# Parcels-code/Parcels

Hardware: AMD Instinct MI355X
Metric: RK4 particle-steps/sec (higher is better)
Workload: dtype f64

## Files before the change

### parcels_amd/csrc/pk_api.hip

```cpp
#include <hip/hip_runtime.h>

#include <algorithm>
#include <array>
#include <chrono>
#include <cmath>
#include <cstdio>
#include <cstdlib>
#include <cstring>
#include <string>
#include <thread>
#include <vector>

#include <rocprim/rocprim.hpp>

#include "pk_hashbuild.h"
#include "pk_neighbors.h"
#include "pk_interact.h"
#include "pk_density.h"
#include "pk_connectivity.h"
#include "pk_host_stage.h"
#include "pk_kernels.h"
#include "pk_ux.h"
#include "pk_sigma.h"

// ... 101 lines not shown
    DCounters* d_counters = nullptr;
    char *d_desc = nullptr, *h_desc = nullptr;
    size_t desc_bytes = 0;
    unsigned long long* d_summary = nullptr;
    void* stage[PK_STAGE_BUFFERS] = {};
    size_t stage_bytes[PK_STAGE_BUFFERS] = {};
    size_t stage_chunk = 0;
    hipEvent_t stage_ev[PK_STAGE_BUFFERS] = {};
    int stage_next = 0;
    double stage_fill_s = 0, stage_wait_s = 0, stage_bytes_total = 0;
    hipDeviceProp_t prop;
    bool in_flight = false;
    int fl_launches = 0;
    int fl_program = 0;
    bool rerun_valid = false;
    pk_exec_params rerun_prm{};
    void (*user_launch)(const void*, int32_t, int32_t, int32_t, uint64_t, void*) = nullptr;
    int32_t user_flags = 0;
    int32_t user_nsample = 0;
    int32_t user_sample_fid[4] = {0, 0, 0, 0};
    char* d_chk = nullptr;
    size_t chk_bytes = 0;
    bool chk_valid = false, chk_has_perm = false;
    int64_t chk_n = 0;
    bool fl_sorted = false;
    int64_t fl_n = 0;
    DCounters* h_counters = nullptr;
    DCounters h_counters0;
    unsigned long long* d_twe = nullptr;
    unsigned long long* d_twe_found = nullptr;
    unsigned int* d_twe_hit = nullptr;
    std::vector<int64_t> twe_found_host;
    std::vector<uint8_t> twe_hit_host;
    bool twe_overflow_host = false;
    int fl_twe_n = 0;
    std::vector<int64_t> rerun_keys;
    unsigned long long* h_summary = nullptr;
    unsigned long long* d_tstats = nullptr;
    unsigned long long* d_clk = nullptr;
    unsigned long long* h_clk = nullptr;
    double* d_sigma = nullptr;
    SigmaA sigma{};
    bool has_sigma = false;
    int sort_horizontal_major = -1;
    int no_special = 0;
    bool eval_points_f32 = false;
    int no_cell_cache = 0;
    int no_hash_dir = 0;
    int no_cell_table = 0;
    int no_fast = 0;
    int no_fast_cgrid = 0;
    bool no_block_cache = false;
    int block_cache = -1;
    int fast_grid = 0;
    struct Snapshot {
        void* dev[PK_NCOLS] = {};
        void* host[PK_NCOLS] = {};
        int64_t capacity = 0;
        int64_t n = 0;
        uint32_t mask = 0;
        int ngrids = 0;
        size_t ss = 0;
        size_t extra_elem[PK_MAX_EXTRA] = {};
        hipEvent_t ready = nullptr, done = nullptr;
        bool in_flight = false;
    } snap[2];
    CoordTable tab_a, tab_c;
    double* d_ct2 = nullptr;
    int ct2_grid = -1;
    int ct2_near = 0;
    char* d_vp = nullptr;
    size_t vp_bytes = 0;
    int vp_fU = -1, vp_fV = -1;
    std::vector<int32_t> vp_level;
    std::vector<uint64_t> vp_gen;
    int clock_probe = 0;
    bool fl_clock_probe = false;
    int no_velocity_pairs = 1;
    uint64_t upload_counter = 0;

    PkSelect sel;
    struct PkComm* comm = nullptr;
    pk::Neighbors* nbr = nullptr;
    pk::Interact* inter = nullptr;

    int32_t fail(const char* where, hipError_t e) {
        err = std::string(where) + ": " + hipGetErrorString(e);
        return -1;
    }
    int32_t fail(const std::string& msg) {
        err = msg;
        return -2;
    }
};

#define PK_HIP(ctx, call)                                  \
    do {                                                   \
        hipError_t e_ = (call);                            \
        if (e_ != hipSuccess) return (ctx)->fail(#call, e_); \
    } while (0)

namespace pk {

PK_DEV unsigned long long order_double(double v) {
    unsigned long long b = (unsigned long long)__double_as_longlong(v);
    return (b & 0x8000000000000000ull) ? ~b : (b | 0x8000000000000000ull);
// ... 402 lines not shown
    }
    pk_ctx* ctx = new pk_ctx();
    ctx->device = device;
    if (const char* e = getenv("PK_SORT_HORIZONTAL")) ctx->sort_horizontal_major = atoi(e);
    if (const char* e = getenv("PK_NO_SPECIAL")) ctx->no_special = atoi(e);
    if (const char* e = getenv("PK_NO_CELL_CACHE")) ctx->no_cell_cache = atoi(e);
    if (const char* e = getenv("PK_NO_HASH_DIR")) ctx->no_hash_dir = atoi(e);
    if (const char* e = getenv("PK_NO_CELL_TABLE")) ctx->no_cell_table = atoi(e);
    if (const char* e = getenv("PK_NO_FAST")) ctx->no_fast = atoi(e);
    if (const char* e = getenv("PK_NO_FAST_CGRID")) ctx->no_fast_cgrid = atoi(e);
    if (const char* e = getenv("PK_NO_VELOCITY_PAIRS")) ctx->no_velocity_pairs = atoi(e);
    if (const char* e = getenv("PK_VELOCITY_PAIRS")) ctx->no_velocity_pairs = !atoi(e);
    ctx->no_block_cache = getenv("PK_NO_BLOCK_CACHE") != nullptr;
    *out = ctx;
    PK_HIP(ctx, hipSetDevice(device));
    PK_HIP(ctx, hipGetDeviceProperties(&ctx->prop, device));
    PK_HIP(ctx, hipStreamCreateWithFlags(&ctx->compute, hipStreamNonBlocking));
    PK_HIP(ctx, hipStreamCreateWithFlags(&ctx->copy, hipStreamNonBlocking));
    PK_HIP(ctx, hipEventCreate(&ctx->ev0));
    PK_HIP(ctx, hipEventCreate(&ctx->ev1));
    PK_HIP(ctx, hipEventCreate(&ctx->ev2));
    PK_HIP(ctx, hipEventCreate(&ctx->ev_p0));
    PK_HIP(ctx, hipEventCreate(&ctx->ev_p1));
    for (int k = 0; k < PK_STAGE_BUFFERS; k++) PK_HIP(ctx, hipEventCreateWithFlags(&ctx->stage_ev[k], hipEventDisableTiming));
    PK_HIP(ctx, hipMalloc((void**)&ctx->d_counters, sizeof(DCounters)));
    PK_HIP(ctx, hipMalloc((void**)&ctx->d_twe, sizeof(unsigned long long) * PK_MAX_TWE));
    PK_HIP(ctx, hipMalloc((void**)&ctx->d_twe_found, sizeof(unsigned long long) * TWE_FOUND_SLOTS));
    PK_HIP(ctx, hipMalloc((void**)&ctx->d_twe_hit, sizeof(unsigned int) * PK_MAX_TWE));
    PK_HIP(ctx, hipMalloc((void**)&ctx->d_summary, sizeof(unsigned long long) * (PK_NUM_STATE_CODES + 2)));
    PK_HIP(ctx, hipHostMalloc((void**)&ctx->h_counters, sizeof(DCounters), hipHostMallocDefault));
    PK_HIP(ctx, hipHostMalloc((void**)&ctx->h_summary, sizeof(unsigned long long) * (PK_NUM_STATE_CODES + 2), hipHostMallocDefault));
    PK_HIP(ctx, hipMalloc((void**)&ctx->d_clk, sizeof(unsigned long long) * 32));
    PK_HIP(ctx, hipMalloc((void**)&ctx->d_tstats, sizeof(unsigned long long) * 3));
    PK_HIP(ctx, hipHostMalloc((void**)&ctx->h_clk, sizeof(unsigned long long) * 32, hipHostMallocDefault));
    return 0;
}

int32_t pk_set_option(pk_ctx* ctx, const char* name, int32_t value) {
    if (!ctx || !name) return -2;
    const std::string n(name);
    if (n == "fast_path") ctx->no_fast = !value;
    else if (n == "fast_cgrid") ctx->no_fast_cgrid = !value;
    else if (n == "velocity_pairs") ctx->no_velocity_pairs = !value;
    else if (n == "clock_probe") ctx->clock_probe = value;
    else if (n == "special_programs") ctx->no_special = !value;
    else if (n == "cell_cache") ctx->no_cell_cache = !value;
    else if (n == "hash_directory") ctx->no_hash_dir = !value;
    else if (n == "cell_table") ctx->no_cell_table = !value;
    else if (n == "sort_horizontal") ctx->sort_horizontal_major = value;
    else if (n == "eval_points_f32") ctx->eval_points_f32 = value != 0;
    else if (n == "block_cache") {
        if (value < -1 || value > 2) return ctx->fail("pk_set_option: block_cache is -1 (planned), 0 (none), 1 (stage-pair block) or 2 (level-pair cache)");
        ctx->block_cache = value;
    }
    else if (n == "fast_grid") {
        if (value < 0) return ctx->fail("pk_set_option: fast_grid is 0 (planned) or the largest number of workgroups of the persistent A-grid launch");
        ctx->fast_grid = value;
    }
    else return ctx->fail("pk_set_option: unknown option '" + n + "'");
    return 0;
}

int32_t pk_upload_stats(pk_ctx* ctx, double* out4) {
    if (!ctx || !out4) return -2;
    out4[0] = ctx->stage_fill_s;
    out4[1] = ctx->stage_wait_s;
    out4[2] = ctx->stage_bytes_total;
    out4[3] = (double)pkhost::copy_threads();
    return 0;
}

static void free_snapshots(pk_ctx* ctx) {
    for (auto& sn : ctx->snap) {
        if (sn.in_flight && sn.done) (void)hipEventSynchronize(sn.done);
        for (int k = 0; k < PK_NCOLS; k++) {
            if (sn.dev[k]) (void)hipFree(sn.dev[k]);
            if (sn.host[k]) (void)hipHostFree(sn.host[k]);
            sn.dev[k] = sn.host[k] = nullptr;
        }
        sn.capacity = 0;
        sn.in_flight = false;
    }
}

int32_t pk_destroy(pk_ctx* ctx) {
    if (!ctx) return 0;
    (void)hipSetDevice(ctx->device);
    (void)hipDeviceSynchronize();
    for (auto& g : ctx->grids)
        for (void* p : g.allocs) (void)hipFree(p);
    for (auto& f : ctx->fields) {
        if (f.dev_data && f.owns_data) (void)hipFree(f.dev_data);
        if (f.dev_time) (void)hipFree(f.dev_time);
    }
    free_particles(ctx);
    free_snapshots(ctx);
    for (auto& sn : ctx->snap) {
        if (sn.ready) (void)hipEventDestroy(sn.ready);
        if (sn.done) (void)hipEventDestroy(sn.done);
    }
    if (ctx->d_pack_tmp) (void)hipFree(ctx->d_pack_tmp);
    if (ctx->tab_a.d) (void)hipFree(ctx->tab_a.d);
    if (ctx->tab_c.d) (void)hipFree(ctx->tab_c.d);
    if (ctx->d_ct2) (void)hipFree(ctx->d_ct2);
    if (ctx->d_vp) (void)hipFree(ctx->d_vp);
    if (ctx->d_sigma) (void)hipFree(ctx->d_sigma);
// ... 1556 lines not shown
    const bool sigma_module = us.present && (us.flags & PK_USER_SIGMA);
    if (sigma_module && !croco && !ctx->has_sigma)
        return ctx->fail("the registered user program was built for the CROCO sigma loop: it runs a list on a context with CROCO parameters only (pk_set_croco)");
    if (croco || sigma_module) {
        if (!ctx->has_sigma) return ctx->fail("a CROCO kernel needs the CROCO parameters of the context (pk_set_croco)");
        if (us.present && !sigma_module)
            return ctx->fail("the registered user program was built for the kernel-list interpreter: a list with a CROCO kernel needs the sigma variant (PK_USER_SIGMA)");
        if (ctx_is_typed(ctx)) return ctx->fail("the CROCO kernels need float64 coordinate arrays");
        if (prm->interp_uv != 0 && prm->interp_uv != 1) return ctx->fail("the CROCO program interpolates the velocity with XLinear_Velocity or CGrid_Velocity");
        p.prog = PROG_SIGMA;
        p.lds = (size_t)ctx->sigma.n * 2 * sizeof(double);
        a.sigma = ctx->sigma;
        return 0;
    }
    bool rest_policy = true;
    for (int k = 1; k < prm->nk; k++)
        rest_policy = rest_policy && (prm->kernels[k] == PK_KERNEL_DELETE_ON_ERROR || prm->kernels[k] == PK_KERNEL_DELETE_OUT_OF_BOUNDS);
    if (rest_policy && use_lds) {
        if (prm->kernels[0] == PK_KERNEL_ADVECTION_RK4) p.prog = PROG_RK4;
        if (prm->kernels[0] == PK_KERNEL_ADVECTION_RK4_3D) p.prog = PROG_RK4_3D;
        if (prm->kernels[0] == PK_KERNEL_ADVECTION_RK45 && !ctx->no_special) p.prog = PROG_RK45;
        if (prm->kernels[0] == PK_KERNEL_ADVECTIONDIFFUSION_M1 && !ctx->no_special) p.prog = PROG_M1;
    }
    if (prm->body_only) p.prog = PROG_GENERIC;
    const bool typed = ctx_is_typed(ctx);
    if (typed) p.prog = PROG_TYPED;
    const bool curv = ctx->grids[a.main_grid].d.kind == 1;
    const bool listed = prm->twe_n > 0 && !us.assume_unlisted;
    const int ufast = (us.present && use_lds && !listed && !typed) ? user_fast_shape(prm, us.flags) : -1;
    const bool user_samples = us.nsample > 0 || (us.flags & (PK_USER_SAMPLES_UV | PK_USER_SAMPLES_UVW));
    int fast_prog = -1;
    const bool ride = ufast >= 0 && (!curv || !user_samples);
    if (ride) fast_prog = ufast ? PROG_RK4_3D : PROG_RK4;
    else if (!listed && (p.prog == PROG_RK4 || p.prog == PROG_RK4_3D || (curv && (p.prog == PROG_RK45 || p.prog == PROG_M1)))) fast_prog = p.prog;
    if (fast_prog < 0) return 0;
    if (!curv) {
        if (int32_t rc = fill_fast(ctx, prm, a, fast_prog)) return rc;
        if (ride && a.fast.ok && !fill_fast_scalars(ctx, prm, a.fast, us.nsample, us.fids)) a.fast.ok = 0;
        if (!a.fast.ok) return 0;
        p.kernel = fast_prog == PROG_RK4_3D ? DEDICATED_A3 : DEDICATED_A2;
        p.lds = (size_t)a.fast.lds_n * 2 * sizeof(double);
        const bool lp_kernel = fast_prog == PROG_RK4 && !ride;
        const size_t lp_lds = (p.lds + (size_t)FAST_LP_BYTES + 2047) / 2048 * 2048;
        const bool lp_fits = 2 * lp_lds <= (size_t)160 * 1024;
        int mode = ctx->block_cache;
        if (ctx->no_block_cache && mode != 2) mode = 0;
        if (mode == 2 && !(lp_kernel && lp_fits))
            return ctx->fail(!lp_kernel ? "block_cache 2: only the library's 2-D A-grid kernel (AdvectionRK4 without user kernels) has the level-pair cache"
                                        : "block_cache 2: the coordinate tables leave no room for the level-pair cache at 16 waves per CU");
        if (mode < 0) mode = lp_kernel && lp_fits ? 2 : 1;
        if (mode == 2) {
            p.lp = FAST_LP_CACHE;
            a.fast.lds_blk = a.fast.lds_n;
            p.lds += (size_t)FAST_LP_BYTES;
        } else if (mode == 0 && lp_kernel && !ctx->no_block_cache) {
            p.lp = FAST_LP_REGS;
            a.fast.lds_blk = 0;
        } else {
            const bool blk = mode == 1 && fast_prog != PROG_RK4_3D && p.lds + (size_t)FAST_BLK_BYTES <= 64 * 1024;
            a.fast.lds_blk = blk ? a.fast.lds_n : 0;
            if (blk) p.lds += (size_t)FAST_BLK_BYTES;
        }
    } else {
        if (int32_t rc = fill_fastc(ctx, prm, a, fast_prog, prm->have_guess0 || us.assume_guessed, p.lds)) return rc;
        if (!a.fastc.ok) return 0;
        p.kernel = fast_prog == PROG_RK4_3D ? DEDICATED_C3 : DEDICATED_C2;
    }
    p.prog = fast_prog;
    p.ride = ride;
    return 0;
}

static void launch_general(int prog, int field_f32, int curv, const pk_exec_params* prm, int use_lds, const KArgs& a, dim3 grid, size_t lds_bytes, hipStream_t s) {
    switch (prog) {
        case PROG_RK4: launch_program<PROG_RK4>(field_f32, curv, prm->interp_uv, use_lds, a, grid, lds_bytes, s); break;
        case PROG_RK4_3D: launch_program<PROG_RK4_3D>(field_f32, curv, prm->interp_uv, use_lds, a, grid, lds_bytes, s); break;
        case PROG_RK45: launch_program<PROG_RK45>(field_f32, curv, prm->interp_uv, use_lds, a, grid, lds_bytes, s); break;
        case PROG_M1: launch_program<PROG_M1>(field_f32, curv, prm->interp_uv, use_lds, a, grid, lds_bytes, s); break;
        case PROG_TYPED: launch_program<PROG_TYPED>(field_f32, curv, prm->interp_uv, use_lds, a, grid, lds_bytes, s); break;
        default: launch_program<PROG_GENERIC>(field_f32, curv, prm->interp_uv, use_lds, a, grid, lds_bytes, s); break;
    }
}

int32_t pk_execute_begin(pk_ctx* ctx, const pk_exec_params* prm) {
    if (!ctx || !prm) return -2;
    if (!ctx->bound) return ctx->fail("no particles bound");
    if (ctx->in_flight) return ctx->fail("pk_execute_begin: a launch is already in flight (call pk_execute_end)");
    if (prm->nk < 1 || prm->nk > PK_MAX_KERNELS) return ctx->fail("params.nk out of range");
    PK_HIP(ctx, hipSetDevice(ctx->device));
    ctx->fl_clock_probe = false;
    KArgs a;
    size_t lds_bytes = 0;
    int use_lds = 0;
    int32_t rc = launch_args(ctx, prm, a, lds_bytes, use_lds);
    if (rc) return rc;
    rc = upload_descriptors(ctx, a);
    if (rc) return rc;
    bool need_kh = false, has_user = false;
    for (int k = 0; k < prm->nk; k++) {
        const int id = prm->kernels[k];
        if (id == PK_KERNEL_ADVECTIONDIFFUSION_M1 || id == PK_KERNEL_ADVECTIONDIFFUSION_EM || id == PK_KERNEL_DIFFUSION_UNIFORM_KH)
            need_kh = true;
        if (id == PK_KERNEL_ADVECTION_RK45 && !ctx->dev.next_dt) return ctx->fail("AdvectionRK45 needs the next_dt column");
        if (id >= PK_KERNEL_USER0 && id < PK_KERNEL_USER0 + PK_MAX_USER_KERNELS) {
            has_user = true;
            if (!ctx->user_launch) return ctx->fail("a user kernel id without a registered program (pk_set_user_program)");
// ... 813 lines not shown
```

### parcels_amd/csrc/pk_device.h

```cpp
#pragma once
#include <hip/hip_runtime.h>
#include <stdint.h>

#include "../../include/parcels_hip.h"

namespace pk {

struct DGrid {
    int32_t kind, spherical;
    int32_t has_x, has_y, has_z;
    int32_t nx, ny, nz;
    int32_t xdim, ydim, zdim;
    int32_t off_x, off_y, off_z;
    int32_t lon_f32, lat_f32, depth_f32;
    int32_t h_bitwidth;
    double deg2m;
    const double* lon;
    const double* lat;
    const double* depth;
    const double* node_tab;
    const double* cell_tab;
    const uint32_t* h_keys;
    const int64_t* h_starts;
    const int64_t* h_counts;
// ... 21 lines not shown
};

struct DParticles {
    int64_t n;
    int32_t ngrids, spatial_f32;
    double* t;
    void *z, *y, *x, *dz, *dy, *dx;
    double* dt;
    double* next_dt;
    int32_t* state;
    int32_t* ei;
    int64_t* particle_id;
    void* extra[PK_MAX_EXTRA];
    int32_t extra_f32[PK_MAX_EXTRA];
    int32_t* iter;
};

struct DPOut {
    double* t;
    void *z, *y, *x, *dz, *dy, *dx;
    double* dt;
    double* next_dt;
    int32_t* state;
    int32_t* ei;
    int32_t* iter;
};

struct DCounters {
    unsigned long long steps, attempts, paused;
    unsigned int err_iter, pad;
    unsigned long long twe_key;
    unsigned int twe_overflow, pad2;
    unsigned int pad3[20];
    unsigned int cursor[8 * 32];
};
constexpr int PK_CURSOR_STRIDE = 32;
static_assert(offsetof(DCounters, cursor) == 128, "the cursors start on a line of their own");

struct FastA {
    int32_t ok, grid;
    int32_t has_ti, has_z, has_y, has_x, spherical;
    int32_t nt, nslots;
    int32_t gnz, gny, gnx;
    uint32_t ex, ey, ez;
    uint32_t st_z, st_y;
    uint32_t dyb, dzb;
    int32_t lds_time, lds_depth, lds_lat, lds_lon, lds_n;
    int32_t lds_blk;
    int64_t lvl_b;
    const char *U, *V, *W;
    const double* tab;
    double tlen, t0, t1, z0, z1, y0, y1, x0, x1;
    double deg2m, inv_deg2m;
    int32_t ns, pad1;
    int32_t sfid[4];
    const char* S[4];
};

struct FastC {
    int32_t ok, grid;
    int32_t has_ti, has_z, walk_ok, near_edges;
    int32_t nt, nslots;
    int32_t gnz, gny, gnx;
    uint32_t ex, ey, ez;
    int32_t lds_time, lds_depth, lds_n;
    int32_t lds_rec, lds_fv;
    int32_t st_z, st_y;
    int32_t cb;
    int64_t lvl_b;
    int64_t dU0, dU1, dV0, dV1;
    union { int64_t dW0; int64_t vp_slot_b; };
    union { int64_t dW1; int64_t vp_hi; };
    const char *U, *V;
    union { const char* W; const char* vp; };
    const char* kh[2];
    int32_t kh_st[2], kh_sz[2], kh_sy[2];
    int32_t kh_nt[2], kh_nz[2], kh_ny[2], kh_nx[2], kh_has_ti[2], kh_nslots[2];
    const double* ct2;
    const double* tab;
    double tlen, t0, t1, z0, z1, deg2m;
};

struct SigmaA {
    const double* tab;
    int32_t n;
    int32_t fh, fzeta;
    int32_t cs_f32;
    double hc;
};

#define PK_CONST_AS __attribute__((address_space(4)))
struct KArgs {
    const PK_CONST_AS DGrid* grids;
    const PK_CONST_AS DField* fields;
    DParticles p;
    pk_exec_params prm;
    double win_lo, win_hi;
    DCounters* counters;
    const unsigned long long* twe_listed;
    unsigned long long* twe_found;
    unsigned int* twe_hit;
    int32_t lds_time, lds_depth, lds_lat, lds_lon, lds_total;
    int32_t lds_cc_nodes, lds_cc_keys, lds_cc_fvals;
    int32_t main_grid, main_field;
    DPOut po;
    union {
        FastA fast;
// ... 1417 lines not shown
```

### parcels_amd/csrc/pk_fast_agrid.h

```cpp
#pragma once
#include "pk_device.h"

namespace pk {

typedef double pk_tab2 __attribute__((ext_vector_type(2)));

struct FastTabs {
    const pk_tab2* time;
    const pk_tab2* depth;
    const pk_tab2* lat;
    const pk_tab2* lon;
    pk_tab2* blk;
    uint32_t fl;
    double tlen;
    int32_t gny, gnx;
    double deg2m, inv_deg2m;
};
PK_DEV void pin_scalars(FastTabs& T, const FastA& F) {
    T.tlen = F.tlen;
    T.gny = F.gny;
    T.gnx = F.gnx;
#ifdef PK_FAST_PIN
    asm volatile("" : "+s"(T.tlen), "+s"(T.gny), "+s"(T.gnx));
#endif
// ... 299 lines not shown
    lp_field<FT, LT, LZ>(fu, F.U + o0, F.U + o1, bo, F.dyb, F.dzb, zeta);
    lp_field<FT, LT, LZ>(fv, F.V + o0, F.V + o1, bo, F.dyb, F.dzb, zeta);
}
PK_DEV double lp_sum(const LpField& f, double tau, double eta, double xsi) {
    const double p0 = fma(tau, f.d0.x, f.p0.x), px = fma(tau, f.d0.y, f.p0.y), py = fma(tau, f.d1.x, f.p1.x), pxy = fma(tau, f.d1.y, f.p1.y);
    return fma(eta, fma(xsi, pxy, py), fma(xsi, px, p0));
}

PK_DEV double fma3(double a, double b, double c) {
    double r;
    asm("v_fma_f64 %0, %1, %2, %3" : "=v"(r) : "v"(a), "v"(b), "v"(c));
    return r;
}
PK_DEV double lp_sum_held(const LpField& f, double tau, double eta, double xsi) {
    const double p0 = fma3(tau, f.d0.x, f.p0.x), px = fma3(tau, f.d0.y, f.p0.y), py = fma3(tau, f.d1.x, f.p1.x), pxy = fma3(tau, f.d1.y, f.p1.y);
    return fma(eta, fma(xsi, pxy, py), fma(xsi, px, p0));
}

PK_DEV int uniform_i32(int v) { return __builtin_amdgcn_readfirstlane(v); }

#ifndef PK_FAST_CELL_REGS
#define PK_FAST_CELL_REGS 1
#endif
constexpr bool fast_cell_regs(int lp) { return PK_FAST_CELL_REGS != 0 && lp == FAST_LP_CACHE; }

#ifndef PK_FAST_BLOCK_REGS
#define PK_FAST_BLOCK_REGS 1
#endif
constexpr bool fast_block_regs(int lp, bool pf) { return PK_FAST_BLOCK_REGS != 0 && fast_cell_regs(lp) && !pf; }
#ifndef PK_FAST_TIME_REC
#define PK_FAST_TIME_REC 1
#endif
constexpr bool fast_time_rec(int lp, bool pf) { return PK_FAST_TIME_REC != 0 && fast_block_regs(lp, pf); }

#ifndef PK_FAST_WSUM
#define PK_FAST_WSUM 1
#endif
#ifndef PK_FAST_CONV_STEP
#define PK_FAST_CONV_STEP 1
#endif
#ifdef PK_USER_KERNELS
constexpr bool fast_wsum(int, bool) { return false; }
constexpr bool fast_conv_step(int, bool) { return false; }
#else
constexpr bool fast_wsum(int lp, bool pf) { return PK_FAST_WSUM != 0 && fast_block_regs(lp, pf); }
constexpr bool fast_conv_step(int lp, bool pf) { return PK_FAST_CONV_STEP != 0 && fast_block_regs(lp, pf); }
#endif
PK_DEV double fma3s(double wgt, double b, double c) {
    double r;
    asm("v_fma_f64 %0, %1, %2, %3" : "=v"(r) : "s"(wgt), "v"(b), "v"(c));
    return r;
}

PK_DEV int fast_oob_state(int s, int xi, int yi, int zi, double xsi, double eta, double zeta, double tau) {
    if ((xi == RIGHT_OUT_OF_BOUNDS || yi == RIGHT_OUT_OF_BOUNDS || zi == RIGHT_OUT_OF_BOUNDS) && s < PK_ERROROUTOFBOUNDS) s = PK_ERROROUTOFBOUNDS;
    if (zi == LEFT_OUT_OF_BOUNDS && s < PK_ERRORTHROUGHSURFACE) s = PK_ERRORTHROUGHSURFACE;
    const bool bad = !(isfinite(xsi) && isfinite(eta) && isfinite(zeta) && isfinite(tau));
    if (bad && s < PK_ERRORINTERPOLATION) s = PK_ERRORINTERPOLATION;
    return s;
}

struct FCtx {
    int state;
    int32_t ei;
    int ht, hz, hy, hx;
    int zi;
    uint32_t zez;
    double mt, mtau, mz, mzeta;
    int32_t bei;
    int32_t bkey;
    double ya, yb, yr, xa, xb, xr;
    LpField fu, fv;
    double ta, tb, tr;
};
constexpr int32_t FAST_NO_BLOCK = -0x7fffffff - 1;
constexpr int FAST_Z_UNSEARCHED = -3;
constexpr int FAST_Z_UNSEARCHED_PACKED = -0x7fffffff - 1;
PK_DEV void fctx_depth_moved(FCtx& c, bool packed = false) {
    c.zi = packed ? FAST_Z_UNSEARCHED_PACKED : FAST_Z_UNSEARCHED;
    c.ya = __builtin_inf();
}
PK_DEV void fctx_init(FCtx& c, int state, int32_t ei, bool cell_regs = false, bool packed = false) {
    c.state = state;
    c.ei = ei;
    c.ht = c.hz = c.hy = c.hx = 0;
    c.zi = packed ? FAST_Z_UNSEARCHED_PACKED : cell_regs ? FAST_Z_UNSEARCHED : 0;
    c.ya = c.xa = c.ta = __builtin_inf();
    c.yb = c.xb = c.yr = c.xr = c.tb = c.tr = 0.0;
    c.zez = 0u;
    c.mt = c.mz = __builtin_nan("");
    c.mtau = c.mzeta = 0.0;
    c.bei = FAST_NO_BLOCK;
    c.bkey = -1;
    c.fu.p0 = c.fu.p1 = c.fu.d0 = c.fu.d1 = c.fv.p0 = c.fv.p1 = c.fv.d0 = c.fv.d1 = pk_tab2{0.0, 0.0};
}

template <class FT, bool PF, bool D3, int LP = FAST_LP_OFF>
PK_DEV void eval_uvw_fast(const KArgs& a, const FastTabs& T, FCtx& c, double t, double z, double y, double x, bool pos_f32, double& u,
                          double& v, double& w, unsigned it, int klo, int bmode = 0) {
    const FastA& F = a.fast;
    uint32_t fl = T.fl;
    asm volatile("" : "+s"(fl));
    u = v = w = 0.0;
    constexpr bool BR = fast_block_regs(LP, PF);
    constexpr bool SPEC = fast_cell_regs(LP) && !PF && !BR;
    LpField fu, fv;
// ... 77 lines not shown
        } else {
            CellEntries e;
            if (yx2) {
                fast_search2(T.lat, T.gny, F.y0, F.y1, y, c.hy, yi, eta, T.lon, T.gnx, F.x0, F.x1, x, c.hx, xi, xsi, &e);
            } else {
                if (fl & FA_Y) fast_search<true>(T.lat, T.gny, F.y0, F.y1, y, c.hy, yi, eta, (fl & FA_NY2) != 0);
                if (fl & FA_X) fast_search<true>(T.lon, T.gnx, F.x0, F.x1, x, c.hx, xi, xsi, (fl & FA_NX2) != 0);
            }
            c.ei = (int32_t)((uint32_t)xi + (uint32_t)yi * F.ey + (BR ? (uint32_t)zi * F.ez : c.zez));
            if (__builtin_expect((xi | yi | zi) < 0, 0)) {
                if (BR) zeta = depth_zeta();
                c.state = fast_oob_state(c.state, xi, yi, zi, xsi, eta, zeta, tau);
                c.ya = __builtin_inf();
                return;
            }
            if (yx2) {
                c.ya = e.ea.x; c.yb = e.a1a; c.yr = e.ea.y;
                c.xa = e.eb.x; c.xb = e.a1b; c.xr = e.eb.y;
            }
        }
    } else {
        if (PK_FAST_SEARCH2 && (fl & YX2) == YX2) {
            fast_search2(T.lat, T.gny, F.y0, F.y1, y, c.hy, yi, eta, T.lon, T.gnx, F.x0, F.x1, x, c.hx, xi, xsi);
        } else {
            if (fl & FA_Y) fast_search<true>(T.lat, T.gny, F.y0, F.y1, y, c.hy, yi, eta, (fl & FA_NY2) != 0);
            if (fl & FA_X) fast_search<true>(T.lon, T.gnx, F.x0, F.x1, x, c.hx, xi, xsi, (fl & FA_NX2) != 0);
        }
        c.ei = (int32_t)((uint32_t)xi + __umul24((uint32_t)yi, F.ey) + c.zez);
        if (__builtin_expect((xi | yi | zi) < 0, 0)) {
            c.ei = (int32_t)((uint32_t)xi + (uint32_t)yi * F.ey + c.zez);
            int s = c.state;
            if ((xi == RIGHT_OUT_OF_BOUNDS || yi == RIGHT_OUT_OF_BOUNDS || zi == RIGHT_OUT_OF_BOUNDS) && s < PK_ERROROUTOFBOUNDS) s = PK_ERROROUTOFBOUNDS;
            if (zi == LEFT_OUT_OF_BOUNDS && s < PK_ERRORTHROUGHSURFACE) s = PK_ERRORTHROUGHSURFACE;
            const bool bad = !(isfinite(xsi) && isfinite(eta) && isfinite(zeta) && isfinite(tau));
            if (bad && s < PK_ERRORINTERPOLATION) s = PK_ERRORINTERPOLATION;
            c.state = s;
            return;
        }
    }
    const bool lenT = tau > 0, lenZ = BR ? (c.zi & 1) != 0 : !(zeta <= 0);
    const int key = (ti << 2) | (lenT ? 2 : 0) | (!BR && lenZ ? 1 : 0);
    if (CR) { yi = c.hy; xi = c.hx; }
    const uint32_t b00 = ((uint32_t)zi * F.st_z + (uint32_t)yi * F.st_y + (uint32_t)xi) * (uint32_t)sizeof(FT);
    const double omt = 1 - tau, omz = 1 - zeta, omx = 1 - xsi, ome = 1 - eta;
    const double w00 = omx * ome, w01 = xsi * ome, w10 = omx * eta, w11 = xsi * eta;
    double uu = 0.0, vv = 0.0, ww = 0.0;
    if constexpr (LP != FAST_LP_OFF) {
        static_assert(!D3, "the level-pair arithmetic is the 2-D kernel's (z must not move)");
        const bool miss = LP == FAST_LP_REGS || c.ei != c.bei || key != c.bkey;
        const bool some_miss = LP == FAST_LP_REGS || __builtin_amdgcn_ballot_w64(miss) != 0;
        if (some_miss) {
            if (BR) zeta = depth_zeta();
            const int wkey = BR ? key | (lenZ ? 1 : 0) : key;
            for (bool done = !miss; !done;) {
                const int uk = uniform_i32(wkey);
                const int uti = uk >> 2;
                int s0 = uti, s1 = uti + 1;
                if (fl & FA_RING) {
                    s0 = (int)((uint32_t)s0 % (uint32_t)F.nslots);
                    s1 = (int)((uint32_t)s1 % (uint32_t)F.nslots);
                }
                int64_t o0 = (int64_t)s0 * F.lvl_b, o1 = (int64_t)s1 * F.lvl_b;
                int lens = uk & 3;
                asm volatile("" : "+s"(o0), "+s"(o1), "+s"(lens));
                if (wkey == uk) {
                    if (lens == 3) lp_fetch<FT, true, true>(F, o0, o1, b00, zeta, fu, fv);
                    else if (lens == 2) lp_fetch<FT, true, false>(F, o0, o1, b00, zeta, fu, fv);
                    else if (lens == 1) lp_fetch<FT, false, true>(F, o0, o1, b00, zeta, fu, fv);
                    else lp_fetch<FT, false, false>(F, o0, o1, b00, zeta, fu, fv);
                    done = true;
                }
            }
            if (LP == FAST_LP_CACHE && miss) {
                T.blk[0] = fu.p0; T.blk[FAST_WG_LP] = fu.p1; T.blk[2 * FAST_WG_LP] = fu.d0; T.blk[3 * FAST_WG_LP] = fu.d1;
                T.blk[4 * FAST_WG_LP] = fv.p0; T.blk[5 * FAST_WG_LP] = fv.p1; T.blk[6 * FAST_WG_LP] = fv.d0; T.blk[7 * FAST_WG_LP] = fv.d1;
                c.bei = c.ei;
                c.bkey = key;
            }
        }
        if constexpr (BR) {
            if (some_miss) {
                c.fu.p0 = T.blk[0]; c.fu.p1 = T.blk[FAST_WG_LP]; c.fu.d0 = T.blk[2 * FAST_WG_LP]; c.fu.d1 = T.blk[3 * FAST_WG_LP];
                c.fv.p0 = T.blk[4 * FAST_WG_LP]; c.fv.p1 = T.blk[5 * FAST_WG_LP]; c.fv.d0 = T.blk[6 * FAST_WG_LP]; c.fv.d1 = T.blk[7 * FAST_WG_LP];
            }
            uu = lp_sum_held(c.fu, tau, eta, xsi);
            vv = lp_sum_held(c.fv, tau, eta, xsi);
        } else {
            if (LP == FAST_LP_CACHE && (!SPEC || some_miss)) {
                fu.p0 = T.blk[0]; fu.p1 = T.blk[FAST_WG_LP]; fu.d0 = T.blk[2 * FAST_WG_LP]; fu.d1 = T.blk[3 * FAST_WG_LP];
                fv.p0 = T.blk[4 * FAST_WG_LP]; fv.p1 = T.blk[5 * FAST_WG_LP]; fv.d0 = T.blk[6 * FAST_WG_LP]; fv.d1 = T.blk[7 * FAST_WG_LP];
            }
            uu = lp_sum(fu, tau, eta, xsi);
            vv = lp_sum(fv, tau, eta, xsi);
        }
    } else {
        const bool bc = !D3 && PK_FAST_BLOCK_CACHE && (fl & FA_BLK) != 0;
        bool reuse = false;
        if (bc && (bmode & 1)) reuse = __builtin_amdgcn_ballot_w64(c.ei != c.bei) == 0;
        if (reuse) {
            const pk_tab2 b0 = T.blk[0], b1 = T.blk[FAST_WG], b2 = T.blk[2 * FAST_WG], b3 = T.blk[3 * FAST_WG];
            uu = w00 * b0.x + w01 * b0.y + w10 * b1.x + w11 * b1.y;
            vv = w00 * b2.x + w01 * b2.y + w10 * b3.x + w11 * b3.y;
        } else {
            const bool keep = bc && (bmode & 2);
            pk_tab2* const blk = keep ? T.blk : nullptr;
            for (bool done = false; !done;) {
                const int uk = uniform_i32(key);
                const int uti = uk >> 2;
                int s0 = uti, s1 = uti + 1;
                if (fl & FA_RING) {
                    s0 = (int)((uint32_t)s0 % (uint32_t)F.nslots);
                    s1 = (int)((uint32_t)s1 % (uint32_t)F.nslots);
                }
                int64_t o0 = (int64_t)s0 * F.lvl_b, o1 = (int64_t)s1 * F.lvl_b;
                int lens = uk & 3;
                asm volatile("" : "+s"(o0), "+s"(o1), "+s"(lens));
                if (key == uk) {
                    if (lens == 3) uvw_fast<FT, D3, true, true>(F, o0, o1, b00, tau, omt, zeta, omz, w00, w01, w10, w11, uu, vv, ww, blk);
                    else if (lens == 2) uvw_fast<FT, D3, true, false>(F, o0, o1, b00, tau, omt, zeta, omz, w00, w01, w10, w11, uu, vv, ww, blk);
                    else if (lens == 1) uvw_fast<FT, D3, false, true>(F, o0, o1, b00, tau, omt, zeta, omz, w00, w01, w10, w11, uu, vv, ww, blk);
                    else uvw_fast<FT, D3, false, false>(F, o0, o1, b00, tau, omt, zeta, omz, w00, w01, w10, w11, uu, vv, ww, blk);
                    done = true;
                }
            }
            if (keep) c.bei = c.ei;
        }
// ... 96 lines not shown
```

### parcels_amd/csrc/pk_kernels.h

```cpp
#pragma once
#include "pk_device.h"
#include "pk_fast_agrid.h"
#include "pk_fast_cgrid.h"

namespace pk {

static_assert(sizeof(KArgs) <= 4096, "kernel arguments must fit the 4 KiB kernarg segment");

enum Program { PROG_RK4 = 0, PROG_RK4_3D = 1, PROG_GENERIC = 2, PROG_RK45 = 3, PROG_M1 = 4, PROG_TYPED = 5 };

struct PState {
    double t, z, y, x, dz, dy, dx, dt, next_dt;
    int64_t id;
};

PK_DEV double ldp(const void* col, int64_t i, bool pf) { return pf ? (double)((const float*)col)[i] : ((const double*)col)[i]; }
PK_DEV void stp(void* col, int64_t i, double v, bool pf) {
    if (pf) ((float*)col)[i] = (float)v; else ((double*)col)[i] = v;
}
PK_DEV double padd(bool pf, double a, double b) { return pf ? (double)((float)a + (float)b) : a + b; }
PK_DEV double psub(bool pf, double a, double b) { return pf ? (double)((float)a - (float)b) : a - b; }
PK_DEV double pstore(bool pf, double v) { return pf ? (double)(float)v : v; }

enum { RQ_UV = 0, RQ_UVW = 1, RQ_SCALAR = 2 };
// ... 610 lines not shown
    c.state = fc.state;
    c.pf = PF;
    c.row = row;
    c.hz = c.hy = c.hx = c.ht = 0;
    c.hyx_valid = false;
    c.first_eval = 0u;
    c.u32 = c.v32 = c.oob = false;
    c.ei0 = c.ei1 = c.ei2 = c.ei3 = 0;
    c.it = it;
    c.klo = kslot * 1000;
    c.zpos_f32 = false;
    KLocal L;
    Request rq;
#pragma unroll 1
    for (int stage = 0; !user_prepare(a, kid - PK_KERNEL_USER0, stage, kslot, c, p, L, rq); stage++) {
        double u = 0.0, v = 0.0, w = 0.0;
        fc.state = c.state;
        if (rq.kind == RQ_SCALAR) {
            int slot = 0;
            for (int k = 1; k < a.fast.ns; k++) slot = a.fast.sfid[k] == rq.fidx ? k : slot;
            u = eval_scalar_fast<FT, PF>(a, ft, fc, slot, rq.t, rq.z, rq.y, rq.x, it, kslot * 1000 + stage);
        } else {
            eval_uvw_fast<FT, PF, D3>(a, ft, fc, rq.t, rq.z, rq.y, rq.x, PF && rq.f32, u, v, w, it, kslot * 1000 + stage);
        }
        c.state = fc.state;
        L.r[3] = u; L.r[4] = v; L.r[5] = w;
    }
    t = p.t; z = p.z; y = p.y; x = p.x; dz = p.dz; dy = p.dy; dx = p.dx; dt = p.dt;
    fc.state = c.state;
}
#endif

#ifndef PK_MIN_WAVES_FAST
#define PK_MIN_WAVES_FAST 4
#endif
template <class FT, int PFM, bool D3, int LP = FAST_LP_OFF>
__global__ void __launch_bounds__(fast_wg(LP), PK_MIN_WAVES_FAST) advect_fast_kernel(const KArgs a) {
    extern __shared__ __attribute__((aligned(16))) double smem[];
    constexpr int WG = fast_wg(LP);
    FastTabs ft;
    {
        pk_tab2* s_tab = reinterpret_cast<pk_tab2*>(smem);
        const pk_tab2* g_tab = reinterpret_cast<const pk_tab2*>(a.fast.tab);
        for (int k = threadIdx.x; k < a.fast.lds_n; k += WG) s_tab[k] = g_tab[k];
        __syncthreads();
        ft.time = s_tab + a.fast.lds_time;
        ft.depth = s_tab + a.fast.lds_depth;
        ft.lat = s_tab + a.fast.lds_lat;
        ft.lon = s_tab + a.fast.lds_lon;
        ft.blk = s_tab + a.fast.lds_blk + threadIdx.x;
        pin_scalars(ft, a.fast);
        ft.fl = fast_flags(a.fast) | ((a.win_lo > -INFINITY || a.win_hi < INFINITY) ? FA_WIN : 0u) | (a.prm.dt0 > 0 ? FA_FWD : 0u) |
                (a.prm.max_iters > 0 ? FA_MAXIT : 0u);
    }
    constexpr bool PERS = fast_persistent(LP);
    [[maybe_unused]] unsigned chunk = 0u, tried = 0u;
    [[maybe_unused]] const unsigned nchunks = PERS ? (unsigned)((a.p.n + FAST_CHUNK - 1) / FAST_CHUNK) : 0u;
    auto row = [&]() {
        if constexpr (PERS) {
            unsigned tid = threadIdx.x;
            asm volatile("" : "+v"(tid));
            return (int64_t)chunk * FAST_CHUNK + (tid & 63u);
        } else return (int64_t)xcd_swizzle(blockIdx.x, gridDim.x) * WG + threadIdx.x;
    };
    [[maybe_unused]] unsigned long long all_steps = 0ull, all_attempts = 0ull, all_paused = 0ull;
    do {
        if constexpr (PERS) {
            if (!fast_claim(a.counters, nchunks, tried, chunk)) break;
        }
        unsigned steps = 0, attempts = 0, paused = 0;
        if (row() < a.p.n) {
            int64_t i = row();
            const DParticles& P = a.p;
            const DPOut& O = a.po;
            const pk_exec_params& prm = a.prm;
            constexpr bool pf = PFM == 1;
            FCtx c;
            c.state = prm.reset_state ? PK_EVALUATE : P.state[i];
            if (c.state == PK_EVALUATE) {
                unsigned it = prm.reset_state ? 0u : (unsigned)P.iter[i];
                fctx_init(c, PK_EVALUATE, P.ei[i * P.ngrids + a.fast.grid], fast_cell_regs(LP), fast_block_regs(LP, pf));
                double pt = P.t[i];
                double pz = ldp(P.z, i, pf), py = ldp(P.y, i, pf), px = ldp(P.x, i, pf);
                double pdz = ldp(P.dz, i, pf), pdy = ldp(P.dy, i, pf), pdx = ldp(P.dx, i, pf);
                double pdt = P.dt[i];
                const double endtime = prm.endtime;
                while (c.state == PK_EVALUATE) {
                    uint32_t fl = ft.fl;
                    asm volatile("" : "+s"(fl));
                    if constexpr (fast_conv_step(LP, pf)) {
                        ft.deg2m = a.fast.deg2m;
                        ft.inv_deg2m = a.fast.inv_deg2m;
                        asm volatile("" : "+s"(ft.deg2m), "+s"(ft.inv_deg2m));
                    }
                    const bool fwd = (fl & FA_FWD) != 0;
                    const double tte = fwd ? endtime - pt : -(endtime - pt);
                    if (!(tte >= 0)) break;
                    if ((fl & FA_MAXIT) && it >= (unsigned)prm.max_iters) break;
                    double dtc;
                    if (fwd) dtc = fmax(fmin(pdt, tte), 0.0);
                    else dtc = fmin(fmax(pdt, -tte), 0.0);
                    if (fl & FA_WIN) {
                        const double t1 = pt + dtc;
                        const double lo = fmin(pt, t1), hi = fmax(pt, t1);
                        if (lo < a.win_lo || hi > a.win_hi) { paused = 1; break; }
                    }
// ... 706 lines not shown
```

Baseline: 51.00 billion.

## Transpose sparse level-pair cache misses across wavefront lanes for cooperative fetch

When only a few lanes of a wavefront miss the level-pair LDS cache, the missing cells are spread across the lanes: each lane loads one corner pair for one missing cell. The depth and time interpolation and differencing are then done with DPP lane swizzles, and the results are written into the missing lanes' LDS cache slots. This replaces the serial per-unique-key refill loop, which runs once per distinct miss and leaves most lanes idle. It adds bpermute and DPP overhead and a new option, miss_lanes (default 4), that caps how many missing lanes take this path.

After: 52.37 billion (median of 6 runs). 1.03x the previous value.

```diff
diff --git a/parcels_amd/csrc/pk_api.hip b/parcels_amd/csrc/pk_api.hip
--- a/parcels_amd/csrc/pk_api.hip
+++ b/parcels_amd/csrc/pk_api.hip
@@ -177,6 +177,7 @@
     int no_fast_cgrid = 0;
     bool no_block_cache = false;
     int block_cache = -1;
+    int miss_lanes = -1;
     int fast_grid = 0;
     struct Snapshot {
         void* dev[PK_NCOLS] = {};
@@ -685,6 +686,10 @@
     else if (n == "block_cache") {
         if (value < -1 || value > 2) return ctx->fail("pk_set_option: block_cache is -1 (planned), 0 (none), 1 (stage-pair block) or 2 (level-pair cache)");
         ctx->block_cache = value;
+    }
+    else if (n == "miss_lanes") {
+        if (value < -1 || value > 64) return ctx->fail("pk_set_option: miss_lanes is -1 (planned), 0 (never) or the most missing lanes of a wavefront, up to 64");
+        ctx->miss_lanes = value;
     }
     else if (n == "fast_grid") {
         if (value < 0) return ctx->fail("pk_set_option: fast_grid is 0 (planned) or the largest number of workgroups of the persistent A-grid launch");
@@ -2347,6 +2352,7 @@
         if (mode == 2) {
             p.lp = FAST_LP_CACHE;
             a.fast.lds_blk = a.fast.lds_n;
+            a.fast.miss_lanes = ctx->miss_lanes < 0 ? FAST_MISS_LANES_DEFAULT : ctx->miss_lanes;
             p.lds += (size_t)FAST_LP_BYTES;
         } else if (mode == 0 && lp_kernel && !ctx->no_block_cache) {
             p.lp = FAST_LP_REGS;
diff --git a/parcels_amd/csrc/pk_device.h b/parcels_amd/csrc/pk_device.h
--- a/parcels_amd/csrc/pk_device.h
+++ b/parcels_amd/csrc/pk_device.h
@@ -97,7 +97,8 @@
     const double* tab;
     double tlen, t0, t1, z0, z1, y0, y1, x0, x1;
     double deg2m, inv_deg2m;
-    int32_t ns, pad1;
+    int32_t ns;
+    int32_t miss_lanes;
     int32_t sfid[4];
     const char* S[4];
 };
diff --git a/parcels_amd/csrc/pk_fast_agrid.h b/parcels_amd/csrc/pk_fast_agrid.h
--- a/parcels_amd/csrc/pk_fast_agrid.h
+++ b/parcels_amd/csrc/pk_fast_agrid.h
@@ -375,6 +375,90 @@
     return r;
 }
 
+#ifndef PK_FAST_MISS_XPOSE
+#define PK_FAST_MISS_XPOSE 1
+#endif
+#ifdef PK_USER_KERNELS
+constexpr bool fast_miss_xpose(int, bool) { return false; }
+#else
+constexpr bool fast_miss_xpose(int lp, bool pf) { return PK_FAST_MISS_XPOSE != 0 && fast_block_regs(lp, pf); }
+#endif
+constexpr int FAST_MISS_LANES_DEFAULT = 4;
+constexpr uint32_t FA_MISS_LANES_SHIFT = 16u;
+constexpr int DPP_XOR1 = 0xB1, DPP_XOR2 = 0x4E, DPP_SHR4 = 0x114;
+template <int CTRL, int BANKS>
+PK_DEV double dpp_f64(double v) {
+    const uint64_t b = __builtin_bit_cast(uint64_t, v);
+    const int lo = (int)(uint32_t)b, hi = (int)(uint32_t)(b >> 32);
+    uint32_t rlo, rhi;
+    if constexpr (BANKS == 0xf) {
+        rlo = (uint32_t)__builtin_amdgcn_mov_dpp(lo, CTRL, 0xf, 0xf, true);
+        rhi = (uint32_t)__builtin_amdgcn_mov_dpp(hi, CTRL, 0xf, 0xf, true);
+    } else {
+        rlo = (uint32_t)__builtin_amdgcn_update_dpp(lo, lo, CTRL, 0xf, BANKS, false);
+        rhi = (uint32_t)__builtin_amdgcn_update_dpp(hi, hi, CTRL, 0xf, BANKS, false);
+    }
+    return __builtin_bit_cast(double, (uint64_t)rlo | ((uint64_t)rhi << 32));
+}
+PK_DEV void ldpair_at(uint64_t addr, double& a, double& b, double) {
+    const pk_double2 v = *reinterpret_cast<const __attribute__((address_space(1))) pk_double2*>((uintptr_t)addr);
+    a = v.x;
+    b = v.y;
+}
+PK_DEV void ldpair_at(uint64_t addr, double& a, double& b, float) {
+    const pk_float2 v = *reinterpret_cast<const __attribute__((address_space(1))) pk_float2*>((uintptr_t)addr);
+    a = (double)v.x;
+    b = (double)v.y;
+}
+PK_DEV uint32_t lane_u32(uint32_t v, int src) { return (uint32_t)__builtin_amdgcn_ds_bpermute(src << 2, (int)v); }
+template <class FT>
+PK_DEV void lp_fetch_xposed(const FastA& F, const FastTabs& T, uint64_t mm, int wkey, uint32_t b00, double zeta) {
+    uint32_t lane = __builtin_amdgcn_mbcnt_hi(~0u, __builtin_amdgcn_mbcnt_lo(~0u, 0u));
+    const uint64_t zb = __builtin_bit_cast(uint64_t, zeta);
+    const uint32_t kb = 0u - (lane & 1u), rb = 0u - ((lane >> 1) & 1u), fb = 0u - ((lane >> 3) & 1u);
+    const uint64_t du = (uint64_t)(uintptr_t)F.U, dv = (uint64_t)(uintptr_t)F.V - du;
+    uint64_t fbase = du + ((uint64_t)((uint32_t)dv & fb) | ((uint64_t)((uint32_t)(dv >> 32) & fb) << 32));
+    uint64_t rowoff = (uint64_t)(F.dzb & kb) + (uint64_t)(F.dyb & rb);
+    uint32_t lvl_b = (uint32_t)F.lvl_b;
+    asm volatile("" : "+v"(fbase), "+v"(rowoff), "+v"(lvl_b), "+v"(lane));
+    do {
+        uint32_t four = 0u;
+        for (int q = 0; q < 4; q++) {
+            four |= (mm ? (uint32_t)__builtin_ctzll(mm) : 0xffu) << (8 * q);
+            mm &= mm - 1;
+        }
+        uint32_t ln = lane;
+        asm volatile("" : "+v"(ln));
+        const uint32_t m = (four >> ((ln >> 4) * 8u)) & 0xffu;
+        const int src = (int)(m & 63u);
+        const uint32_t mb00 = lane_u32(b00, src), mkey = lane_u32((uint32_t)wkey, src);
+        const double mzeta = __builtin_bit_cast(double, (uint64_t)lane_u32((uint32_t)zb, src) | ((uint64_t)lane_u32((uint32_t)(zb >> 32), src) << 32));
+        const uint32_t lbit = (ln >> 2) & 1u;
+        const uint64_t addr = fbase + ((uint64_t)((mkey >> 2) + lbit) * (uint64_t)lvl_b + rowoff + (uint64_t)mb00);
+        const uint32_t skip = (m >> 7) | (ln & 1u & ~mkey) | (lbit & ~(mkey >> 1));
+        double cx = 0.0, cy = 0.0;
+        if (skip == 0u) ldpair_at(addr, cx, cy, FT());
+        const double dx = dpp_f64<DPP_XOR1, 0xf>(cx), dy = dpp_f64<DPP_XOR1, 0xf>(cy);
+        const double zx = fma(mzeta, dx - cx, cx), zy = fma(mzeta, dy - cy, cy);
+        const bool lenZ = (mkey & 1u) != 0;
+        cx = lenZ ? zx : cx;
+        cy = lenZ ? zy : cy;
+        const double ax = dpp_f64<DPP_SHR4, 0xa>(cx), ay = dpp_f64<DPP_SHR4, 0xa>(cy);
+        const bool lenT = (mkey & 2u) != 0;
+        const double ex = lenT ? cx - ax : 0.0, ey = lenT ? cy - ay : 0.0;
+        const bool l = lbit != 0;
+        cx = l ? ex : cx;
+        cy = l ? ey : cy;
+        const double h = cy - cx;
+        const double ox = dpp_f64<DPP_XOR2, 0xf>(cx), oh = dpp_f64<DPP_XOR2, 0xf>(h);
+        const bool r = (ln & 2u) != 0;
+        pk_tab2 e;
+        e.x = r ? cx - ox : cx;
+        e.y = r ? h - oh : h;
+        if (((m >> 7) | (ln & 1u)) == 0u) (T.blk + ((int)m - (int)ln))[((ln >> 1) & 7u) * FAST_WG_LP] = e;
+    } while (mm);
+}
+
 PK_DEV int fast_oob_state(int s, int xi, int yi, int zi, double xsi, double eta, double zeta, double tau) {
     if ((xi == RIGHT_OUT_OF_BOUNDS || yi == RIGHT_OUT_OF_BOUNDS || zi == RIGHT_OUT_OF_BOUNDS) && s < PK_ERROROUTOFBOUNDS) s = PK_ERROROUTOFBOUNDS;
     if (zi == LEFT_OUT_OF_BOUNDS && s < PK_ERRORTHROUGHSURFACE) s = PK_ERRORTHROUGHSURFACE;
@@ -558,7 +642,20 @@
         if (some_miss) {
             if (BR) zeta = depth_zeta();
             const int wkey = BR ? key | (lenZ ? 1 : 0) : key;
-            for (bool done = !miss; !done;) {
+            [[maybe_unused]] bool xposed = false;
+            if constexpr (fast_miss_xpose(LP, PF)) {
+                const uint64_t mm = __builtin_amdgcn_ballot_w64(miss);
+                xposed = __builtin_amdgcn_ballot_w64(true) == ~0ull && !(fl & FA_RING) &&
+                         (uint32_t)__builtin_popcountll(mm) <= ((fl >> FA_MISS_LANES_SHIFT) & 127u);
+                if (xposed) {
+                    lp_fetch_xposed<FT>(F, T, mm, wkey, b00, zeta);
+                    if (miss) {
+                        c.bei = c.ei;
+                        c.bkey = key;
+                    }
+                }
+            }
+            for (bool done = !miss || xposed; !done;) {
                 const int uk = uniform_i32(wkey);
                 const int uti = uk >> 2;
                 int s0 = uti, s1 = uti + 1;
@@ -577,7 +674,7 @@
                     done = true;
                 }
             }
-            if (LP == FAST_LP_CACHE && miss) {
+            if (LP == FAST_LP_CACHE && miss && !xposed) {
                 T.blk[0] = fu.p0; T.blk[FAST_WG_LP] = fu.p1; T.blk[2 * FAST_WG_LP] = fu.d0; T.blk[3 * FAST_WG_LP] = fu.d1;
                 T.blk[4 * FAST_WG_LP] = fv.p0; T.blk[5 * FAST_WG_LP] = fv.p1; T.blk[6 * FAST_WG_LP] = fv.d0; T.blk[7 * FAST_WG_LP] = fv.d1;
                 c.bei = c.ei;
diff --git a/parcels_amd/csrc/pk_kernels.h b/parcels_amd/csrc/pk_kernels.h
--- a/parcels_amd/csrc/pk_kernels.h
+++ b/parcels_amd/csrc/pk_kernels.h
@@ -686,6 +686,7 @@
         pin_scalars(ft, a.fast);
         ft.fl = fast_flags(a.fast) | ((a.win_lo > -INFINITY || a.win_hi < INFINITY) ? FA_WIN : 0u) | (a.prm.dt0 > 0 ? FA_FWD : 0u) |
                 (a.prm.max_iters > 0 ? FA_MAXIT : 0u);
+        if constexpr (fast_miss_xpose(LP, PFM == 1)) ft.fl |= (uint32_t)a.fast.miss_lanes << FA_MISS_LANES_SHIFT;
     }
     constexpr bool PERS = fast_persistent(LP);
     [[maybe_unused]] unsigned chunk = 0u, tried = 0u;
```
